# dmsuehir/unet_distributed

Hardware: AMD Instinct MI355X
Metric: images/sec (whole node) 2D UNet BraTS 128×128×4 at 1/2/4/8 MI355X; Dice parity (higher is better)
Workload: dtype bf16; 1 GPU; model=unet2d-transposed (base 32, depth 4, 7760385 params), global_batch=1024, per_gpu_batch=1024, img_size=128, in_channels=4, parallelism=dp1, backend=native

## Files before the change

unet_distributed_amd/csrc/kernels/conv_dw.hip:

```cpp
#include "common.h"
#include "conv_params.h"
#include "conv_epilogue.h"
#include "conv_win.h"
#include "head_grad.h"

namespace unet {
namespace {

constexpr int DW_NTHR = 256;
constexpr int DW_W = 128, DW_R = 2, DW_HR = DW_R + 2, DW_BM = DW_W * DW_R, DW_BN = 32;
constexpr int DW_HWP = (DW_W + 2 + 15) / 16 * 16;
constexpr int DW_PPR = DW_HWP / 16;
constexpr int DW_ROWB = DW_HWP * 64;
constexpr int DW_XI = DW_HR * DW_PPR;
constexpr int DW_WI = 9 * DW_BN / 16;
constexpr int DW_AI = DW_BM / 16;
constexpr int DW_WB = DW_WI * 1024, DW_XB = DW_XI * 1024, DW_AB = DW_AI * 1024;
constexpr int DW_KB = 6 * 32 * 4;
constexpr int DW_LDS = DW_WB + DW_XB + DW_AB + DW_KB;
static_assert(DW_BM * 64 + 4 * 2 * DW_BN * 4 <= 2 * DW_ROWB, "epilogue staging aliases two halo rows");
static_assert(4 * 64 * 16 * 4 <= DW_LDS, "slab reduction scratch");
constexpr int DW_HG = DW_HR * DW_HWP * 4;
constexpr int DW_HJ = DW_HG / DW_NTHR;
static_assert(DW_HG == DW_HJ * DW_NTHR, "whole granule passes");

template <int XF>
__device__ __forceinline__ void dw_dlogit(const ConvFwdParams& p, const float (&pr)[DW_HJ], const float (&tv)[DW_HJ],
                                          float (&dl)[DW_HJ]) {
  if constexpr (XF == 4) {
    const float I = p.hg.sums[0], St = p.hg.sums[1], Sp = p.hg.sums[2];
    const float a = -2.f / (2.f * I + 1.f), bb = 1.f / (St + Sp + 1.f);
    const float gs = p.hg.gscale ? *p.hg.gscale : 1.f;
#pragma unroll
    for (int j = 0; j < DW_HJ; ++j) dl[j] = head_dlogit(pr[j], tv[j], a, bb, p.hg.inv_total, p.hg.bce_w, gs);
  } else {
    const float gs = p.hg.gscale ? *p.hg.gscale : 1.f;
    const float al = -2.f * gs / (2.f * p.hg.sums[0] + 1.f);
    const float be = gs / (p.hg.sums[1] + p.hg.sums[2] + 1.f);
    const float ga = gs * p.hg.bce_w * p.hg.inv_total;
#pragma unroll
    for (int j = 0; j < DW_HJ; ++j) dl[j] = hn_dlogit(pr[j], tv[j], al, be, ga);
  }
}

template <int EPI, int XF, bool SEG = false>
__global__ void __launch_bounds__(DW_NTHR, 2) conv_dw_kernel(const ConvFwdParams p) {
  static_assert(XF == 0 || XF == 2 || XF == 3 || XF == 4,
                "plain dY, norm backward on load (of the normalised head), head gradient on load");
  constexpr int W = DW_W, R = DW_R, HR = DW_HR, ROWB = DW_ROWB, BN = DW_BN;
  constexpr int TM = 4, TN = 2, TC = 2, RW = 2, NCS = 4;
  __shared__ __attribute__((aligned(1024))) char smem[DW_LDS];
  char* Ws = smem;
  char* Xs = smem + DW_WB;
  char* As = Xs + DW_XB;

  const int tid = threadIdx.x, lane = tid & 63, wave = __builtin_amdgcn_readfirstlane(tid >> 6);
  const int H = p.OH;
  const int rows_total = p.N * H;
  const int Wf = SEG ? p.OW : W;
  const int M = rows_total * Wf;
  const int nrp = rows_total / R;
  const int nwin = nrp * (SEG ? Wf / W : 1);
  const int split = blockIdx.x;
  const int w_begin = (int)((long long)split * nwin / p.fw.nsplit);
  const int w_end = (int)((long long)(split + 1) * nwin / p.fw.nsplit);
  constexpr int OOB = 0x7fffffff;
  const int C = p.C1;
  const int Cx = p.fw.Cx;
  const int lslot = lane >> 2;
  const int lchunk = (lane & 3) ^ ((lslot >> 1) & 3);
  const int fsub = lane >> 4, fr = lane & 15;
  const int c0 = wave * 32;
  static_assert(DW_HR == 4 && DW_AI % 4 == 0, "one halo row per wave");
  const int dma_lane = ((lslot - 1) * 32 + lchunk * 8) * 2;
  const int xdma_lane = (lslot * 32 + lchunk * 8) * 2;

  {
    const __amdgpu_buffer_rsrc_t rsw = __builtin_amdgcn_make_buffer_rsrc((void*)p.wgt, (short)0, OOB, 0x00020000);
    const int wl = (lslot * p.Kpad + lchunk * 8) * 2;
#pragma unroll
    for (int q = 0; q < (DW_WI + 3) / 4; ++q) {
// ... 18 lines not shown
  const int G = lane >> 4, tq = (lane >> 2) & 3, pp = lane & 3;
  const int jw = wave & 1, sw0 = (wave >> 1) * 2;
  auto saddr = [](const int slot, const int col, const int ch) -> int {
    return slot * 64 + (((ch >> 3) ^ ((col >> 1) & 3)) << 4) + ((ch & 7) << 1);
  };
  const int kp0 = 16 * (G >> 1) + 4 * (G & 1) + tq;
  const int abase = saddr(kp0, kp0, 4 * pp);
  int dbase[3];
#pragma unroll
  for (int dw = 0; dw < 3; ++dw) {
    const int hc = kp0 + 2 - dw;
    dbase[dw] = saddr(hc, hc, 4 * pp) ^ (32 * jw);
  }
  auto tr8 = [&](const char* b0, const char* b1) -> h16x8 {
    const short4v lo = __builtin_amdgcn_ds_read_tr16_b64_v4i16(LDS_PTR(short4v, b0));
    const short4v hi = __builtin_amdgcn_ds_read_tr16_b64_v4i16(LDS_PTR(short4v, b1));
    const u32x2 l2 = __builtin_bit_cast(u32x2, lo), h2 = __builtin_bit_cast(u32x2, hi);
    const u32x4 v = {l2[0], l2[1], h2[0], h2[1]};
    return __builtin_bit_cast(h16x8, v);
  };

  f32x4 wacc[9][2];
#pragma unroll
  for (int t = 0; t < 9; ++t)
#pragma unroll
    for (int i = 0; i < 2; ++i) wacc[t][i] = (f32x4){0.f, 0.f, 0.f, 0.f};
  f32x4 bacc = (f32x4){0.f, 0.f, 0.f, 0.f};
  const u32x4 ones_u = {kOnes2, kOnes2, kOnes2, kOnes2};
  const h16x8 ones = __builtin_bit_cast(h16x8, ones_u);
  float* Ks = (float*)(As + DW_AB);
  const int kch = (tid & 3) * 8;
  int fl = 0;

  for (int win = w_begin; win < w_end; ++win) {
    const int seg = SEG ? win / nrp : 0;
    const int col0 = seg * W;
    const int g0 = (SEG ? win - seg * nrp : win) * R;
    const int grow0 = (g0 / H) * H;
    const bool top_in = (g0 % H) != 0, bot_in = ((g0 + R) % H) != 0;
    const bool carry = win > w_begin && top_in;
    if (carry) fl ^= 1;
    const int fo = fl * 2 * ROWB;
    const int k0 = carry ? 2 * DW_HWP * 4 : 0;
    const size_t img_px = (size_t)grow0 * Wf;
    const __amdgpu_buffer_rsrc_t rs1 = __builtin_amdgcn_make_buffer_rsrc(
        (void*)((const char*)p.src1 + img_px * C * 2), (short)0, OOB, 0x00020000);
    const __amdgpu_buffer_rsrc_t rsx = __builtin_amdgcn_make_buffer_rsrc(
        (void*)((const char*)p.fw.x + ((size_t)g0 * Wf + col0) * Cx * 2), (short)0, OOB, 0x00020000);
    u32x4 zv[XF == 2 ? DW_HJ : 1];
    float dl[XF >= 3 ? DW_HJ : 1];
    uint32_t hbits[XF == 4 ? DW_HJ : 1];
    float pr[XF >= 3 ? DW_HJ : 1], tv[XF >= 3 ? DW_HJ : 1];
    uint32_t okm = 0;
    if constexpr (XF >= 2) {
      float kv = 0.f;
      constexpr int NK = XF == 4 ? 32 : XF == 3 ? 192 : 96;
      if (tid < NK) {
        const int m = tid >> 5, c = tid & 31;
        if constexpr (XF == 4) {
          kv = p.hg.w[c];
        } else {
          const float* src = m == 0 ? p.xa : m == 1 ? p.xb : m == 2 ? p.xc : m == 3 ? p.hg.fa : m == 4 ? p.hg.fc : p.xa;
          const size_t ci = (size_t)(g0 / H) * p.xcs + c;
          kv = src[ci];
          if (XF == 3 && m == 5) kv *= p.hg.w[c];
        }
// ... 17 lines not shown
        if constexpr (XF == 2)
          zv[j] = __builtin_amdgcn_raw_buffer_load_b128(rsz, ok ? ((gr - grow0) * Wf + col) * C * 2 + kch * 2 : OOB,
                                                        0, 0);
      }
      if (tid < NK) Ks[tid] = kv;
    }
    __syncthreads();
    if constexpr (XF != 4) {
      const int hr = carry ? 2 + (wave >> 1) : wave;
      const int jlo = carry ? 5 * (wave & 1) : 0, jhi = carry && !(wave & 1) ? 5 : DW_PPR;
      const int gr = g0 - 1 + hr;
      const bool row_ok = (hr > 0 || top_in) && (hr < R + 1 || bot_in) && (unsigned)gr < (unsigned)rows_total;
      const int rowoff = ((gr - grow0) * Wf + col0) * C * 2;
      char* hdst = Xs + (hr ^ (2 * fl)) * ROWB;
#pragma unroll
      for (int j = 0; j < DW_PPR; ++j) {
        if (j < jlo || j >= jhi) continue;
        const bool ok = row_ok && (unsigned)(col0 + 16 * j + lslot - 1) < (unsigned)Wf && 16 * j + lslot <= W + 1;
        const int off = ok ? rowoff + dma_lane + j * 1024 : OOB;
        __builtin_amdgcn_raw_ptr_buffer_load_lds(rs1, (__attribute__((address_space(3))) void*)(hdst + j * 1024),
                                                 16, off, 0, 0, 0);
      }
    }
#pragma unroll
    for (int i = 0; i < DW_AI / 4; ++i) {
      const int k = 4 * wave + i;
      const int xo = SEG ? ((k >> 3) * Wf + 16 * (k & 7)) * Cx * 2 : k * 1024;
      __builtin_amdgcn_raw_ptr_buffer_load_lds(rsx, (__attribute__((address_space(3))) void*)(As + k * 1024), 16,
                                               xdma_lane + xo, 0, 0, 0);
    }
    __syncthreads();
    if constexpr (XF >= 3) dw_dlogit<XF>(p, pr, tv, dl);
    if constexpr (XF == 4) {
      float hw[8];
#pragma unroll
      for (int e = 0; e < 8; ++e) hw[e] = Ks[kch + e];
#pragma unroll
      for (int j = 0; j < DW_HJ; ++j) {
        const int k = k0 + tid + DW_NTHR * j;
        if (k >= DW_HG) continue;
        const int hr = k / (DW_HWP * 4), s = (k >> 2) - hr * DW_HWP;
        float o[8];
#pragma unroll
        for (int e = 0; e < 8; ++e) {
          const float v = dl[j] * hw[e];
          o[e] = ((hbits[j] >> e) & 1u) ? v : 0.f;
        }
        *(u32x4*)(Xs + ((hr ^ (2 * fl)) * DW_HWP + s) * 64 + 16 * ((tid & 3) ^ ((s >> 1) & 3))) = pack8(o);
      }
      __syncthreads();
    } else if constexpr (XF >= 2) {
      float ka[8], kb[8], kc[8], kf[8], kg[8];
#pragma unroll
      for (int e = 0; e < 8; ++e) {
        ka[e] = Ks[(XF == 3 ? 160 : 0) + kch + e];
        kb[e] = Ks[32 + kch + e];
        kc[e] = Ks[64 + kch + e];
        if constexpr (XF == 3) {
          kf[e] = Ks[96 + kch + e];
          kg[e] = Ks[128 + kch + e];
        }
      }
#pragma unroll
      for (int j = 0; j < DW_HJ; ++j) {
        const int k = k0 + tid + DW_NTHR * j;
        if (k >= DW_HG) continue;
        const int hr = k / (DW_HWP * 4), s = (k >> 2) - hr * DW_HWP;
        u32x4* slot = (u32x4*)(Xs + ((hr ^ (2 * fl)) * DW_HWP + s) * 64 + 16 * ((tid & 3) ^ ((s >> 1) & 3)));
        u32x4 v = {0u, 0u, 0u, 0u};
        if ((okm >> j) & 1u) {
          float gf[8], zf[8];
          if constexpr (XF == 3) {
            unpack8(*slot, zf);
#pragma unroll
            for (int e = 0; e < 8; ++e) {
              const float g = fmaf(kf[e], zf[e], kg[e]) > 0.f ? ka[e] * dl[j] : 0.f;
              gf[e] = g + fmaf(kb[e], zf[e], kc[e]);
            }
          } else {
            unpack8(zv[j], zf);
            unpack8(*slot, gf);
#pragma unroll
            for (int e = 0; e < 8; ++e) gf[e] = fmaf(ka[e], gf[e], fmaf(kb[e], zf[e], kc[e]));
          }
          v = pack8(gf);
        }
        *slot = v;
      }
      __syncthreads();
    }

#pragma unroll
    for (int st = 0; st < 2; ++st) {
      const int so = (sw0 + st) * 32 * 64;
      h16x8 xa[R][2];
#pragma unroll
      for (int y = 0; y < R; ++y)
#pragma unroll
        for (int i = 0; i < 2; ++i) {
          const int a = (abase ^ (32 * i)) + y * W * 64 + so;
          xa[y][i] = tr8(As + a, As + a + 512);
        }
#pragma unroll
      for (int hr = 0; hr < HR; ++hr) {
#pragma unroll
        for (int dw = 0; dw < 3; ++dw) {
          const int a = dbase[dw] + hr * ROWB + so + (hr < 2 ? fo : -fo);
          const h16x8 yb = tr8(Xs + a, Xs + a + 512);
          if (dw == 1 && hr >= 1 && hr <= R) bacc = mfma16(ones, yb, bacc);
#pragma unroll
          for (int dh = 0; dh < 3; ++dh) {
            const int y = hr - 2 + dh;
            if (y < 0 || y >= R) continue;
#pragma unroll
            for (int i = 0; i < 2; ++i) wacc[3 * dh + dw][i] = mfma16(xa[y][i], yb, wacc[3 * dh + dw][i]);
          }
        }
        __builtin_amdgcn_sched_barrier(0);
      }
    }

    f32x4 acc[TM][TN];
#pragma unroll
    for (int i = 0; i < TM; ++i)
#pragma unroll
      for (int j = 0; j < TN; ++j) acc[i][j] = (f32x4){0.f, 0.f, 0.f, 0.f};
#pragma unroll
    for (int dw = 0; dw < 3; ++dw) {
      h16x8 wf[3][TN];
#pragma unroll
      for (int dh = 0; dh < 3; ++dh)
#pragma unroll
        for (int j = 0; j < TN; ++j) wf[dh][j] = *(const h16x8*)(Ws + ((3 * dh + dw) * BN + 16 * j) * 64 + wbase);
#pragma unroll
      for (int hr = 0; hr < RW + 2; ++hr) {
#pragma unroll
        for (int ci = 0; ci < TC; ++ci) {
          const h16x8 xf = *(const h16x8*)(Xs + xbase[dw] + hr * ROWB + ci * 16 * 64 + (hr < 2 ? fo : -fo));
#pragma unroll
          for (int dh = 0; dh < 3; ++dh) {
            const int ri = hr - dh;
            if (ri < 0 || ri >= RW) continue;
#pragma unroll
            for (int j = 0; j < TN; ++j) acc[ri * TC + ci][j] = mfma16(wf[dh][j], xf, acc[ri * TC + ci][j]);
          }
        }
      }
    }
    __syncthreads();
    using Map = StripTiles<W, RW, TC, NCS>;
    if constexpr (SEG)
      conv_epilogue<DW_BM, BN, DW_BM / 4, BN, TM, TN, DW_NTHR, EPI, Map, W, W>(p, acc, Xs + fo, g0, 0, M, wave, 0,
                                                                              lane, tid, Wf, col0, win);
    else
      conv_epilogue<DW_BM, BN, DW_BM / 4, BN, TM, TN, DW_NTHR, EPI, Map, 0, W>(p, acc, Xs + fo, g0 * W, 0, M, wave, 0,
                                                                              lane, tid, 0, 0, win);
  }

  float* red = (float*)smem;
  const int row = p.fw.split_lo + split;
  const int n_base = lane & 15, m_base = 4 * (lane >> 4);
  auto reduce_store = [&](const f32x4 (&v4)[2], const int t) {
    __syncthreads();
    if (wave >= 2) {
#pragma unroll
      for (int i = 0; i < 2; ++i) *(f32x4*)(red + ((i * 2 + jw) * 64 + lane) * 4) = v4[i];
    }
    __syncthreads();
    if (wave < 2) {
#pragma unroll
      for (int i = 0; i < 2; ++i) {
        const f32x4 v = v4[i] + *(const f32x4*)(red + ((i * 2 + jw) * 64 + lane) * 4);
        if (t < 9) {
          float* dst = p.fw.slab + (((size_t)row * 9 + t) * Cx + m_base + 16 * i) * C + n_base + 16 * jw;
#pragma unroll
          for (int r = 0; r < 4; ++r) dst[(size_t)r * C] = v[r];
        } else if (i == 0 && lane < 16) {
          p.fw.bias_slab[(size_t)row * C + n_base + 16 * jw] = v[0];
        }
      }
    }
  };
#pragma unroll
  for (int t = 0; t < 9; ++t) reduce_store(wacc[t], t);
  const f32x4 bv[2] = {bacc, (f32x4){0.f, 0.f, 0.f, 0.f}};
  reduce_store(bv, 9);
}

}

const char* conv_dw_check(const ConvFwdParams& p) {
  if (!p.fw.x) return nullptr;
  const int ep = conv_epi_mode(p);
  const bool w_ok = p.OW == DW_W || (p.OW % DW_W == 0 && p.OW <= 8192);
  if (!w_ok || p.IW != p.OW || p.OH != p.IH || p.OH % DW_R || p.KD != 1 || p.OD != 1 || p.ID != 1 ||
      p.KH != 3 || p.KW != 3 || p.stride != 1 || p.pad != 1 || p.C1 != 32 || p.C2 || p.Cout != DW_BN ||
      p.D1 != p.Cout || p.fw.Cx != 32 || (ep != EPI_DGRAD && ep != EPI_DGRAD_NORM) || p.s2d ||
      p.ut.x || p.pool_dst || p.head_w || p.rev)
    return "conv_fwd: fused weight gradient needs a 2D 32 -> 32 channel data gradient on 128-wide rows";
  if (p.xform && (p.xform != 2 || !p.xa || !p.xb || !p.xc || !p.xz || (p.xcs != 0 && p.xcs != p.C1) || p.xout))
    return "conv_fwd: fused weight gradient: norm backward on load (xform 2) needs xa / xb / xc / xz, xcs 0 or C";
  if (p.hg.prob && p.xform && (p.xform != 2 || p.hg.bits || !p.hg.fa || !p.hg.fc || !p.hg.t || !p.hg.sums ||
                                !p.hg.w || p.route_gy))
    return "conv_fwd: fused weight gradient: the normalised head's gradient on load needs xform 2, "
           "fa / fc (no bits), t, sums, w";
  if (p.hg.prob && !p.xform && (!p.hg.bits || !p.hg.t || !p.hg.sums || !p.hg.w || p.route_gy || ep != EPI_DGRAD))
    return "conv_fwd: fused weight gradient: the head gradient on load needs bits, t, sums, w";
  if (!p.fw.slab || !p.fw.bias_slab || p.fw.nsplit < 1 || p.fw.split_lo < 0)
    return "conv_fwd: fused weight gradient needs slab / bias_slab and nsplit >= 1";
  if ((long long)p.OH * p.OW * 32 * 2 >= (1LL << 31) - 64) return "conv_fwd: one image exceeds 2 GiB";
  if (p.OW > DW_W && (p.xform || p.hg.prob || p.nz))
    return "conv_fwd: fused weight gradient on segmented rows: plain dY source, EPI_DGRAD only";
  return nullptr;
}

int conv_dw_grid(const ConvFwdParams& p) { return p.fw.nsplit; }

int conv_dw_stat_rows(const ConvFwdParams& p) { return p.N * p.OH / DW_R; }

hipError_t launch_conv_dw(const ConvFwdParams& p, hipStream_t s) {
  const int ep = conv_epi_mode(p);
  const dim3 grid(p.fw.nsplit), blk(DW_NTHR);
  if (p.OW > DW_W) {
    if (ep != EPI_DGRAD || p.xform || p.hg.prob) return hipErrorInvalidValue;
    UNET_LAUNCH((conv_dw_kernel<EPI_DGRAD, 0, true>), grid, blk, 0, s, p);
  } else if (ep == EPI_DGRAD && !p.xform && !p.hg.prob)
    UNET_LAUNCH((conv_dw_kernel<EPI_DGRAD, 0>), grid, blk, 0, s, p);
  else if (ep == EPI_DGRAD && !p.xform)
    UNET_LAUNCH((conv_dw_kernel<EPI_DGRAD, 4>), grid, blk, 0, s, p);
  else if (ep == EPI_DGRAD && p.xform == 2 && !p.hg.prob)
    UNET_LAUNCH((conv_dw_kernel<EPI_DGRAD, 2>), grid, blk, 0, s, p);
  else if (ep == EPI_DGRAD_NORM && !p.xform && !p.hg.prob)
    UNET_LAUNCH((conv_dw_kernel<EPI_DGRAD_NORM, 0>), grid, blk, 0, s, p);
  else if (ep == EPI_DGRAD_NORM && p.xform == 2 && !p.hg.prob)
    UNET_LAUNCH((conv_dw_kernel<EPI_DGRAD_NORM, 2>), grid, blk, 0, s, p);
  else if (ep == EPI_DGRAD_NORM && p.xform == 2)
    UNET_LAUNCH((conv_dw_kernel<EPI_DGRAD_NORM, 3>), grid, blk, 0, s, p);
  else
    return hipErrorInvalidValue;
  return launch_status();
}

}
```

unet_distributed_amd/csrc/kernels/conv_epilogue.h:

```cpp
#pragma once
#include "common.h"
#include "conv_params.h"

namespace unet {

struct PixCoord {
  int n, d, h, w;
};

__device__ __forceinline__ PixCoord decompose(int q, int OD, int OH, int OW) {
  PixCoord c;
  c.w = q % OW;
  int t = q / OW;
  c.h = t % OH;
  t /= OH;
  c.d = t % OD;
  c.n = t / OD;
  return c;
}

enum { EPI_GENERIC = 0, EPI_FWD = 1, EPI_DGRAD = 2, EPI_STATS = 3, EPI_DGRAD_NORM = 4 };

template <int BM, int BN, int NTHR = 256>
constexpr int epi_lds_bytes() {
// ... 16 lines not shown
}

__host__ __device__ inline const char* conv_norm_epi_check(const ConvFwdParams& p) {
  if (!p.stats && !p.nz) return nullptr;
  if (!p.stats) return "conv_fwd: nz (dgrad-norm epilogue) needs a stats buffer";
  if (p.relu || p.shuffle || p.drop_rate > 0.f || p.out_scale != 1.f || p.D1 != p.Cout || p.mask1 || p.mask2 ||
      p.head_w || p.relu_bits || p.mask_bits || (p.route_gy && !p.nz))
    return "conv_fwd: statistics epilogue takes no ReLU / dropout / shuffle / scale / split / mask / head";
  if (p.nz && (p.bias || !p.na || !p.nc || p.npix <= 0 || p.mask_scale1 != 1.f || (p.ncs != 0 && p.ncs != p.Cout)))
    return "conv_fwd: dgrad-norm epilogue needs na / nc / npix, no bias";
  return nullptr;
}

__host__ __device__ inline int conv_epi_mode(const ConvFwdParams& p) {
  if (p.nz) return EPI_DGRAD_NORM;
  if (p.stats) return EPI_STATS;
  if (p.shuffle || p.drop_rate > 0.f || p.out_scale != 1.f) return EPI_GENERIC;
  if (p.relu && p.D1 == p.Cout && !p.mask1 && !p.mask2 && p.mask_scale1 == 1.f) return EPI_FWD;
  if (!p.relu && !p.bias) return EPI_DGRAD;
  return EPI_GENERIC;
}

template <int WM>
struct LinearTiles {
  __device__ static int base(int wm, int i) { return wm * WM + i * 16; }
};
template <int W, int RW, int TC, int NCS>
struct StripTiles {
  __device__ static int base(int wave, int i) {
    return ((wave / NCS) * RW + i / TC) * W + (wave % NCS) * 16 * TC + (i % TC) * 16;
  }
};

template <int TN>
struct EpiConst {
  float bias[TN][4];
  float hw[8];
  float hb;
};

struct HeadWsum {
  float s[3][8];
  float u, v, w;
};
struct HeadT {
  float t[8];
  bool on;
};

template <int BM, int BN, int WM, int WN, int TM, int TN, int NTHR, int EPI = EPI_GENERIC,
          class MapM = LinearTiles<WM>, int SEGW = 0, int TROW = 0>
__device__ __forceinline__ HeadWsum conv_epilogue(const ConvFwdParams p, f32x4 (&acc)[TM][TN], char* smem,
                                                  const int m0, const int n0, const int M, const int wm,
                                                  const int wn, const int lane, const int tid,
                                                  const int pitch = 0, const int col0 = 0, const int stat_row = 0,
                                                  const EpiConst<TN>* ec = nullptr, const HeadT ht = HeadT{}) {
  HeadWsum hws;
#pragma unroll
  for (int k = 0; k < 3; ++k)
#pragma unroll
    for (int e = 0; e < 8; ++e) hws.s[k][e] = 0.f;
  hws.u = hws.v = hws.w = 0.f;
  auto qof = [&](int ml) -> int {
    if constexpr (SEGW > 0) return (m0 + ml / SEGW) * pitch + col0 + (ml % SEGW);
    else return m0 + ml;
  };
  constexpr bool ESWZ = BN == 32;
  constexpr int EPI_STRIDE = ESWZ ? 64 : (BN + 4) * 2;
  auto eoff = [](const int ml, const int chunk) -> int {
    return ESWZ ? ml * 64 + 16 * (chunk ^ ((ml >> 2) & 3)) : ml * EPI_STRIDE + 16 * chunk;
  };
  auto ehalf = [](const int ml, const int nl) -> int {
    return ESWZ ? ml * 64 + 16 * ((nl >> 3) ^ ((ml >> 2) & 3)) + ((2 * (nl & 7)) ^ (8 * ((ml >> 1) & 1)))
                : ml * EPI_STRIDE + 2 * nl;
  };
  auto eread = [&](const int ml, const int chunk) -> u32x4 {
    if constexpr (ESWZ) {
      const u32x4 v = *(const u32x4*)(smem + eoff(ml, chunk));
      return ((ml >> 1) & 1) ? (u32x4){v[2], v[3], v[0], v[1]} : v;
    } else {
      const u32x2 lo = *(const u32x2*)(smem + eoff(ml, chunk));
      const u32x2 hi = *(const u32x2*)(smem + eoff(ml, chunk) + 8);
      return (u32x4){lo[0], lo[1], hi[0], hi[1]};
    }
  };
  char* E = smem;
  float* SP = (float*)(smem + BM * EPI_STRIDE);
  constexpr bool G = EPI == EPI_GENERIC;
  constexpr bool kNormG = EPI == EPI_DGRAD_NORM;
// ... 23 lines not shown
      for (int i = 0; i < TM; ++i) {
        const int ml = MapM::base(wm, i) + (lane & 15);
        f32x2 a01 = (f32x2){acc[i][j][0], acc[i][j][1]} + b01;
        f32x2 a23 = (f32x2){acc[i][j][2], acc[i][j][3]} + b23;
        u32x2 pk;
        pk[0] = relu2h(pack2h(a01[0], a01[1]));
        pk[1] = relu2h(pack2h(a23[0], a23[1]));
        *(u32x2*)(E + ehalf(ml, nl)) = pk;
      }
      continue;
    }
#pragma unroll
    for (int i = 0; i < TM; ++i) {
      const int ml = MapM::base(wm, i) + (lane & 15);
      const int q = qof(ml);
      float v[4];
#pragma unroll
      for (int r = 0; r < 4; ++r) {
        float x = G ? acc[i][j][r] * p.out_scale + bsv[r] : acc[i][j][r] + bsv[r];
        if (kRelu) x = fmaxf(x, 0.f);
        if (kDrop) {
          const uint32_t h = drop_hash((uint64_t)q * p.Cout + n + r + p.drop_idx0, seed, p.salt);
          x = (h >= drop_thr) ? x * inv_keep : 0.f;
        }
        if (kMaskScale) x *= msc[r];
        v[r] = x;
      }
      u32x2 pk;
      pk[0] = pack2h(v[0], v[1]);
      pk[1] = pack2h(v[2], v[3]);
      *(u32x2*)(E + ehalf(ml, nl)) = pk;
    }
  }
  __syncthreads();

  constexpr int CPR = BN / 8;
  constexpr int NCHUNK = BM * CPR;
  auto stats_out = [&](float (&s1)[8], float (&s2)[8], int cb) {
#pragma unroll
    for (int o = CPR; o < 64; o <<= 1)
#pragma unroll
      for (int e = 0; e < 8; ++e) {
        s1[e] += __shfl_xor(s1[e], o, 64);
        s2[e] += __shfl_xor(s2[e], o, 64);
      }
    const int wv = tid >> 6;
    if ((tid & 63) < CPR) {
#pragma unroll
      for (int e = 0; e < 8; ++e) {
        SP[(wv * 2 + 0) * BN + cb * 8 + e] = s1[e];
        SP[(wv * 2 + 1) * BN + cb * 8 + e] = s2[e];
      }
    }
    __syncthreads();
    for (int t = tid; t < 2 * BN; t += NTHR) {
      const int mom = t / BN, c = t - mom * BN;
      float a = 0.f;
#pragma unroll
      for (int w = 0; w < NTHR / 64; ++w) a += SP[(w * 2 + mom) * BN + c];
      p.stats[((size_t)stat_row * 2 + mom) * p.Cout + n0 + c] = a;
    }
  };
  if constexpr (kStats) {
    static_assert(NCHUNK % NTHR == 0 && NTHR % CPR == 0 && CPR <= 64, "statistics tiling");
    constexpr int NIT = NCHUNK / NTHR, RPI = NTHR / CPR;
    const int cb = tid % CPR, ml0 = tid / CPR;
    const int n = n0 + cb * 8;
// ... 77 lines not shown
        for (int e = 0; e < 8; ++e)
          if (route_hit(cw, e, rk[it], d3)) g[e] += gg[e];
      }
#pragma unroll
      for (int e = 0; e < 8; ++e) {
        bool keep = fmaf(ca[e], z[e], cc[e]) > 0.f;
        if (drop) keep = keep && drop_hash((uint64_t)q * p.Cout + n + e, dseed, p.nd_salt) >= dthr;
        g[e] = keep ? g[e] * dscale : 0.f;
      }
      const u32x4 gv = pack8(g);
      *(u32x4*)(dst + (size_t)q * p.Cout + n) = gv;
      unpack8(gv, g);
#pragma unroll
      for (int e = 0; e < 8; ++e) {
        s1[e] += g[e];
        s2[e] = fmaf(g[e], z[e], s2[e]);
      }
    }
    stats_out(s1, s2, cb);
    return hws;
  }
  if constexpr (EPI == EPI_DGRAD && NCHUNK % NTHR == 0 && NTHR % CPR == 0) {
    constexpr int NIT = NCHUNK / NTHR, RPI = NTHR / CPR;
    const int cb = tid % CPR, ml0 = tid / CPR;
    const int n = n0 + cb * 8;
    const bool side1 = n < p.D1;
    const int rs = side1 ? p.D1 : p.Cout - p.D1;
    const int co = side1 ? n : n - p.D1;
    h16* dst = (h16*)(side1 ? p.dst1 : p.dst2);
    const h16* mk = (const h16*)(side1 ? p.mask1 : p.mask2);
    const bool mbit = (p.mask_bits >> (side1 ? 0 : 1)) & 1;
    u32x4 mv[NIT];
    uint32_t mb[NIT];
    if (mk) {
#pragma unroll
      for (int it = 0; it < NIT; ++it) {
        const int q = qof(ml0 + it * RPI);
        if (q < M) {
          if (mbit)
            mb[it] = ((const uint8_t*)mk)[((size_t)q * rs + co) >> 3];
          else
            mv[it] = *(const u32x4*)(mk + (size_t)q * rs + co);
        }
      }
    }
    const bool route = p.route_gy != nullptr, d3 = p.OD > 1;
    u32x4 rg[NIT];
    uint32_t rc[NIT], rk[NIT];
    if (route) {
      const int cpp = p.Cout >> 3;
#pragma unroll
      for (int it = 0; it < NIT; ++it) {
        const int q = qof(ml0 + it * RPI);
        if (q < M) {
          const size_t pq = route_pix(p, q, rk[it]);
          rc[it] = p.pool_code[pq * cpp + (n >> 3)];
          rg[it] = *(const u32x4*)((const h16*)p.route_gy + pq * p.Cout + n);
        }
      }
    }
#pragma unroll
    for (int it = 0; it < NIT; ++it) {
      const int ml = ml0 + it * RPI;
      const int q = qof(ml);
      if (q >= M) continue;
      u32x4 v = eread(ml, cb);
      if (mk) v = mbit ? keep_bits(v, mb[it]) : keep_pos(v, mv[it]);
      if (route) {
        float o[8], gg[8];
        unpack8(v, o);
        unpack8(rg[it], gg);
        const uint32_t cw = rc[it];
#pragma unroll
        for (int e = 0; e < 8; ++e)
          if (route_hit(cw, e, rk[it], d3)) o[e] += gg[e];
        v = pack8(o);
      }
      *(u32x4*)(dst + (size_t)q * rs + co) = v;
    }
    return hws;
  }
  const int Dt = kShuffle ? (p.Cout >> p.shuffle) : 0;
  constexpr bool kHeadable = EPI == EPI_FWD && BN == 32 && NTHR % CPR == 0;
  const bool kHead = kHeadable && p.head_w != nullptr;
  float hw[8], hb = 0.f;
  constexpr int HIT = kHeadable ? NCHUNK / NTHR : 1;
  static_assert(!kHeadable || (NCHUNK % NTHR == 0 && HIT % CPR == 0 && HIT <= 8), "fused head tiling");
  float hz[HIT];
  int hq[HIT];
#pragma unroll
  for (int k = 0; k < HIT; ++k) {
    hz[k] = 0.f;
    hq[k] = M;
  }
  if (kHeadable && kHead) {
#pragma unroll
    for (int e = 0; e < 8; ++e) hw[e] = ec ? ec->hw[e] : p.head_w[(tid % CPR) * 8 + e];
    hb = ec ? ec->hb : p.head_b[0];
  }
  constexpr int NITER = (NCHUNK + NTHR - 1) / NTHR;
// ... 145 lines not shown
```

unet_distributed_amd/csrc/kernels/conv_params.h:

```cpp
#pragma once
#include <stdint.h>

namespace unet_types {

bool dry_dispatch();

struct HeadGrad {
  const float* prob;
  const void* t;
  const float* sums;
  const float* w;
  const uint8_t* bits;
  const float* gscale;
  float inv_total, bce_w;
  const float* fa;
  const float* fc;
};

struct TconvSrc {
  const void* x;
  const void* w;
  const float* b;
  int C, kpad;
};

struct FusedWgrad {
  const void* x;
  float* slab;
  float* bias_slab;
  int Cx, nsplit, split_lo;
};

struct ConvFwdParams {
  int N, OD, OH, OW;
  int ID, IH, IW;
  int KD, KH, KW, stride, pad;
  int C1, C2;
  int up1;
  const void* src1;
  const void* src2;
  const void* wgt;
  const float* bias;
  int Cout;
  int relu;
  float out_scale;
  float drop_rate;
  uint32_t seed, salt;
  unsigned long long drop_idx0;
  const uint32_t* seed_ptr;
  void* dst1;
  void* dst2;
  int D1;
  const void* mask1;
  const void* mask2;
  float mask_scale1, mask_scale2;
  int shuffle;
  float* stats;
  const void* nz;
  const float* na;
  const float* nc;
  int ncs, npix;
  float nd_rate;
  uint32_t nd_salt;
// ... 128 lines not shown
```

unet_distributed_amd/csrc/runtime/bindings.cpp:

```cpp
#include <pybind11/pybind11.h>
#include <pybind11/stl.h>

#include <functional>
#include <stdexcept>
#include <string>
#include <tuple>
#include <vector>

#include "launch_api.h"

namespace py = pybind11;
using namespace unet;

namespace {

void check(hipError_t e, const char* what) {
  if (e != hipSuccess) throw std::runtime_error(std::string(what) + ": " + hipGetErrorString(e));
}

void check_msg(const char* msg) {
  if (msg) throw std::invalid_argument(msg);
}

template <typename T>
// ... 70 lines not shown
  p.mask_scale2 = get<float>(d, "mask_scale2", 1.f);
  p.shuffle = get<int>(d, "shuffle", 0);
  p.stats = (float*)getp(d, "stats");
  p.nz = getp(d, "nz");
  p.na = (const float*)getp(d, "na");
  p.nc = (const float*)getp(d, "nc");
  p.ncs = get<int>(d, "ncs", 0);
  p.npix = get<int>(d, "npix", 0);
  p.nd_rate = get<float>(d, "nd_rate", 0.f);
  p.nd_salt = get<uint32_t>(d, "nd_salt", 0u);
  p.pool_dst = const_cast<void*>(getp(d, "pool_dst"));
  p.pool_code = (uint32_t*)const_cast<void*>(getp(d, "pool_code"));
  p.relu_bits = (uint8_t*)const_cast<void*>(getp(d, "relu_bits"));
  p.mask_bits = get<int>(d, "mask_bits", 0);
  p.route_gy = getp(d, "route_gy");
  p.xform = get<int>(d, "xform", 0);
  p.xcs = get<int>(d, "xcs", 0);
  p.xa = (const float*)getp(d, "xa");
  p.xb = (const float*)getp(d, "xb");
  p.xc = (const float*)getp(d, "xc");
  p.xz = getp(d, "xz");
  p.s2d = get<int>(d, "s2d", 0);
  p.ut.x = getp(d, "ut_x");
  p.ut.w = getp(d, "ut_w");
  p.ut.b = (const float*)getp(d, "ut_b");
  p.ut.C = get<int>(d, "ut_C", 0);
  p.ut.kpad = get<int>(d, "ut_kpad", 0);
  p.fw.x = getp(d, "fw_x");
  p.fw.slab = (float*)const_cast<void*>(getp(d, "fw_slab"));
  p.fw.bias_slab = (float*)const_cast<void*>(getp(d, "fw_bias_slab"));
  p.fw.Cx = get<int>(d, "fw_Cx", 0);
  p.fw.nsplit = get<int>(d, "fw_nsplit", 0);
  p.fw.split_lo = get<int>(d, "fw_split_lo", 0);
  p.xout = const_cast<void*>(getp(d, "xout"));
  p.xd_rate = get<float>(d, "xd_rate", 0.f);
  p.xd_salt = get<uint32_t>(d, "xd_salt", 0u);
  p.xd_idx0 = get<unsigned long long>(d, "xd_idx0", 0ull);
  p.x2a = (const float*)getp(d, "x2a");
  p.x2b = (const float*)getp(d, "x2b");
  p.x2cs = get<int>(d, "x2cs", 0);
  p.tile = get<int>(d, "tile", 0);
  p.head_w = (const float*)getp(d, "head_w");
  p.head_b = (const float*)getp(d, "head_b");
  p.head_logit = (float*)const_cast<void*>(getp(d, "head_logit"));
  p.head_t = getp(d, "head_t");
  p.head_ws = (float*)const_cast<void*>(getp(d, "head_ws"));
  p.head_nostore = get<int>(d, "head_nostore", 0);
  p.hg = head_grad(d);
  if (!p.src1 || !p.wgt || (!p.dst1 && !(p.head_nostore && p.head_w)))
    throw std::invalid_argument("conv_fwd: src1/wgt/dst1 required");
  check_msg(conv_fwd_prepare(p));
  return p;
}

WgradParams wgrad_params(const py::dict& d) {
  WgradParams p{};
  p.N = get<int>(d, "N", 1);
  p.QD = get<int>(d, "QD", 1);
  p.QH = get<int>(d, "QH", 1);
  p.QW = get<int>(d, "QW", 1);
  p.AD = get<int>(d, "AD", 1);
  p.AH = get<int>(d, "AH", 1);
  p.AW = get<int>(d, "AW", 1);
  p.KD = get<int>(d, "KD", 1);
  p.KH = get<int>(d, "KH", 1);
  p.KW = get<int>(d, "KW", 1);
// ... 803 lines not shown
```

unet_distributed_amd/runtime/native_engine.py:

```python

import math
import os
from contextlib import nullcontext as _nullctx
from typing import Dict, List, Optional, Sequence, Tuple

import numpy as np
import torch

from .. import native
from ..models.spec import UNetSpec
from .params import FlatParams
from .plan_check import RecordingPlan



def _ptr(t: Optional[torch.Tensor]) -> Optional[int]:
    return None if t is None else int(t.data_ptr())


def _r64(k: int) -> int:
    return (k + 63) // 64 * 64


ENGINE_DEFAULTS = dict(dual_stream=1, fwd_streams=2, head_fuse=1, head_onload=1, tconv_fused=2, tconv_wa=1,
                       tconv_onload=1, fwd_offset=6, wg_target=512, dw_fuse=1, dw_wgs=512, win_pf=8, win_cp=1,
                       wg_pair=0, dz_split=0, head_wsum=1, xf_drop=0, wg_pf=1, win_cp3=2, skip_onload=1,
                       route3=1, tail3=0)


class Fusion:

    def __init__(self, doc, norm=None, dims=None, decoder=None, img=None, option=None, needs=(),
                 even_batch=False, cpad=None, when=None):
        self.doc, self.norm, self.dims, self.decoder, self.img = doc, norm, dims, decoder, img
        self.option, self.needs, self.even_batch, self.cpad, self.when = option, tuple(needs), even_batch, cpad, when

    def unmet(self, e) -> List[str]:
        out = []
        if self.norm is not None and e.spec.norm not in self.norm:
            out.append("norm=%s" % e.spec.norm)
        if self.dims is not None and e.dims not in self.dims:
            out.append("dims=%d" % e.dims)
        dec = "upsampling" if e.spec.use_upsampling else "transposed"
        if self.decoder is not None and dec not in self.decoder:
            out.append("decoder=%s" % dec)
        if self.img is not None and e.img not in self.img:
            out.append("img=%d" % e.img)
        if self.option is not None and not e.opts[self.option]:
            out.append("option %s=0" % self.option)
        if self.even_batch and e.B % 2:
            out.append("odd batch")
        if self.cpad is not None and e.cpad not in self.cpad:
            out.append("padded input channels %d" % e.cpad)
        if self.when is not None and not self.when(e):
            out.append("structure")
        return out


_ROW_IMGS = (16, 32, 64, 128)
FUSIONS: Dict[str, Fusion] = {
# ... 636 lines not shown
        b = self.bufs

        def half(t):
            return t.numel() * t.element_size() // 2

        mk = self.relu_bits.get(src1, b[src1]) if d.get("mask1") else None
        h1 = dict(d, N=self.B // 2)
        h2 = dict(h1, src1=d["src1"] + half(dy), dst1=d["dst1"] + half(b["d:" + src1]))
        if mk is not None:
            h2["mask1"] = d["mask1"] + half(mk)
        try:
            for h in (h1, h2):
                self.C.conv_fwd_grid(h)
        except ValueError:
            return None
        self._fusion_on("tail_halves", l.name)
        return h1, h2

    def _plan_dw_fuse(self, l, src1, skip, parts, wspec):
        if (not self._fusion_ok("dw_fused") or skip is not None or l.cin != 32 or l.cout != 32
                or wspec.get("kernel_out") or wspec["kd"].get("xform")
                or wspec["M1"] != 32 or wspec["M2"] or src1 not in self.bufs):
            return None
        nsplit = self.opts["dw_wgs"]
        b = self.bufs
        half = b[src1].numel() * b[src1].element_size() // len(parts)
        if len(parts) > 1 and parts[0].get("nz"):
            return None
        out = []
        for k, d in enumerate(parts):
            if d.get("route_gy") or (d.get("hg_prob") and len(parts) > 1):
                return None
            f = dict(d, rev=0, fw_x=_ptr(b[src1]) + k * half, fw_Cx=l.cin, fw_nsplit=nsplit, fw_split_lo=k * nsplit,
                     name=d["name"])
            if f.get("nz") and not self._restat_dgrad_norm(f, src1):
                return None
            try:
                if self.C.conv_fwd_grid(dict(f, fw_slab=1, fw_bias_slab=1)) != nsplit:
                    return None
            except ValueError:
                return None
            out.append(f)
        wspec["dw"] = dict(rows=nsplit * len(parts))
        self._fusion_on("dw_fused", l.name)
        if len(out) == 1 and l.name in self.norm_layers and self._fusion_ok("dz_onload", l.name):
            C = l.cout
            xf = dict(out[0], xform=2, src1=_ptr(b["d:" + l.name]), xz=_ptr(b["z:" + l.name]),
                      xa=_ptr(b["ca:" + l.name]), xb=_ptr(b["cb:" + l.name]), xc=_ptr(b["cc:" + l.name]),
                      xcs=0 if self.spec.norm == "batch" else C)
            if self._norm_head_loss and l.name == self.head_in:
                hg = self._head_grad_fields()
                hg.pop("hg_bits")
                xf.update(hg, src1=_ptr(b["z:" + l.name]), hg_fa=_ptr(b["fa:" + l.name]),
                          hg_fc=_ptr(b["fc:" + l.name]))
            try:
                ok = self.C.conv_fwd_grid(dict(xf, fw_slab=1, fw_bias_slab=1)) == nsplit
            except ValueError:
                ok = False
            if ok:
                out = [xf]
                self._dz_onload.add(l.name)
                self._fusion_on("dz_onload", l.name)
        return out

    def _dz_split_fields(self, l, src1, skip):
        if (not self._fusion_ok("dz_split") or skip is not None or l.name not in self.norm_layers
                or self.inputs.get(l.name, ("",))[1] != 1 or l.name in self._wa_chain_of
# ... 980 lines not shown
```

Before: 49450 images/sec.

## Software-pipeline fused conv dgrad/wgrad kernel with next-window prefetch

Adds a pipelined variant of the fused weight/data-gradient conv kernel for the plain and head-gradient paths. It issues the next window's input DMA and halo-row (or head probability/target/bit) loads into registers during the current window's MFMA work, replacing full syncthreads with LDS-only barriers. It also preloads mask bits before the compute so the epilogue does not fetch them late. The cost is higher register pressure at 2 waves per SIMD, plus a new code path gated on alignment and routing conditions.

```diff
diff --git a/unet_distributed_amd/csrc/kernels/conv_dw.hip b/unet_distributed_amd/csrc/kernels/conv_dw.hip
--- a/unet_distributed_amd/csrc/kernels/conv_dw.hip
+++ b/unet_distributed_amd/csrc/kernels/conv_dw.hip
@@ -43,10 +43,11 @@
   }
 }
 
-template <int EPI, int XF, bool SEG = false>
+template <int EPI, int XF, bool SEG = false, bool PIPE = false>
 __global__ void __launch_bounds__(DW_NTHR, 2) conv_dw_kernel(const ConvFwdParams p) {
   static_assert(XF == 0 || XF == 2 || XF == 3 || XF == 4,
                 "plain dY, norm backward on load (of the normalised head), head gradient on load");
+  static_assert(!PIPE || (EPI == EPI_DGRAD && (XF == 0 || XF == 4) && !SEG), "variants with a pipelined loop");
   constexpr int W = DW_W, R = DW_R, HR = DW_HR, ROWB = DW_ROWB, BN = DW_BN;
   constexpr int TM = 4, TN = 2, TC = 2, RW = 2, NCS = 4;
   __shared__ __attribute__((aligned(1024))) char smem[DW_LDS];
@@ -131,6 +132,87 @@
   const int kch = (tid & 3) * 8;
   int fl = 0;
 
+  auto wgrad_mfmas = [&](const int fo) {
+#pragma unroll
+    for (int st = 0; st < 2; ++st) {
+      const int so = (sw0 + st) * 32 * 64;
+      h16x8 xa[R][2];
+#pragma unroll
+      for (int y = 0; y < R; ++y)
+#pragma unroll
+        for (int i = 0; i < 2; ++i) {
+          const int a = (abase ^ (32 * i)) + y * W * 64 + so;
+          xa[y][i] = tr8(As + a, As + a + 512);
+        }
+#pragma unroll
+      for (int hr = 0; hr < HR; ++hr) {
+#pragma unroll
+        for (int dw = 0; dw < 3; ++dw) {
+          const int a = dbase[dw] + hr * ROWB + so + (hr < 2 ? fo : -fo);
+          const h16x8 yb = tr8(Xs + a, Xs + a + 512);
+          if (dw == 1 && hr >= 1 && hr <= R) bacc = mfma16(ones, yb, bacc);
+#pragma unroll
+          for (int dh = 0; dh < 3; ++dh) {
+            const int y = hr - 2 + dh;
+            if (y < 0 || y >= R) continue;
+#pragma unroll
+            for (int i = 0; i < 2; ++i) wacc[3 * dh + dw][i] = mfma16(xa[y][i], yb, wacc[3 * dh + dw][i]);
+          }
+        }
+        __builtin_amdgcn_sched_barrier(0);
+      }
+    }
+  };
+  auto dgrad_mfmas = [&](f32x4 (&acc)[TM][TN], const int fo) {
+#pragma unroll
+    for (int i = 0; i < TM; ++i)
+#pragma unroll
+      for (int j = 0; j < TN; ++j) acc[i][j] = (f32x4){0.f, 0.f, 0.f, 0.f};
+#pragma unroll
+    for (int dw = 0; dw < 3; ++dw) {
+      h16x8 wf[3][TN];
+#pragma unroll
+      for (int dh = 0; dh < 3; ++dh)
+#pragma unroll
+        for (int j = 0; j < TN; ++j) wf[dh][j] = *(const h16x8*)(Ws + ((3 * dh + dw) * BN + 16 * j) * 64 + wbase);
+#pragma unroll
+      for (int hr = 0; hr < RW + 2; ++hr) {
+#pragma unroll
+        for (int ci = 0; ci < TC; ++ci) {
+          const h16x8 xf = *(const h16x8*)(Xs + xbase[dw] + hr * ROWB + ci * 16 * 64 + (hr < 2 ? fo : -fo));
+#pragma unroll
+          for (int dh = 0; dh < 3; ++dh) {
+            const int ri = hr - dh;
+            if (ri < 0 || ri >= RW) continue;
+#pragma unroll
+            for (int j = 0; j < TN; ++j) acc[ri * TC + ci][j] = mfma16(wf[dh][j], xf, acc[ri * TC + ci][j]);
+          }
+        }
+      }
+    }
+  };
+  auto form_head_dy = [&](const int k0, const int fl, const auto& dl, const auto& hbits) {
+    if constexpr (XF == 4) {
+      float hw[8];
+#pragma unroll
+      for (int e = 0; e < 8; ++e) hw[e] = Ks[kch + e];
+#pragma unroll
+      for (int j = 0; j < DW_HJ; ++j) {
+        const int k = k0 + tid + DW_NTHR * j;
+        if (k >= DW_HG) continue;
+        const int hr = k / (DW_HWP * 4), s = (k >> 2) - hr * DW_HWP;
+        float o[8];
+#pragma unroll
+        for (int e = 0; e < 8; ++e) {
+          const float v = dl[j] * hw[e];
+          o[e] = ((hbits[j] >> e) & 1u) ? v : 0.f;
+        }
+        *(u32x4*)(Xs + ((hr ^ (2 * fl)) * DW_HWP + s) * 64 + 16 * ((tid & 3) ^ ((s >> 1) & 3))) = pack8(o);
+      }
+    }
+  };
+
+  if constexpr (!PIPE)
   for (int win = w_begin; win < w_end; ++win) {
     const int seg = SEG ? win / nrp : 0;
     const int col0 = seg * W;
@@ -214,22 +296,7 @@
     __syncthreads();
     if constexpr (XF >= 3) dw_dlogit<XF>(p, pr, tv, dl);
     if constexpr (XF == 4) {
-      float hw[8];
-#pragma unroll
-      for (int e = 0; e < 8; ++e) hw[e] = Ks[kch + e];
-#pragma unroll
-      for (int j = 0; j < DW_HJ; ++j) {
-        const int k = k0 + tid + DW_NTHR * j;
-        if (k >= DW_HG) continue;
-        const int hr = k / (DW_HWP * 4), s = (k >> 2) - hr * DW_HWP;
-        float o[8];
-#pragma unroll
-        for (int e = 0; e < 8; ++e) {
-          const float v = dl[j] * hw[e];
-          o[e] = ((hbits[j] >> e) & 1u) ? v : 0.f;
-        }
-        *(u32x4*)(Xs + ((hr ^ (2 * fl)) * DW_HWP + s) * 64 + 16 * ((tid & 3) ^ ((s >> 1) & 3))) = pack8(o);
-      }
+      form_head_dy(k0, fl, dl, hbits);
       __syncthreads();
     } else if constexpr (XF >= 2) {
       float ka[8], kb[8], kc[8], kf[8], kg[8];
@@ -272,63 +339,9 @@
       __syncthreads();
     }
 
-#pragma unroll
-    for (int st = 0; st < 2; ++st) {
-      const int so = (sw0 + st) * 32 * 64;
-      h16x8 xa[R][2];
-#pragma unroll
-      for (int y = 0; y < R; ++y)
-#pragma unroll
-        for (int i = 0; i < 2; ++i) {
-          const int a = (abase ^ (32 * i)) + y * W * 64 + so;
-          xa[y][i] = tr8(As + a, As + a + 512);
-        }
-#pragma unroll
-      for (int hr = 0; hr < HR; ++hr) {
-#pragma unroll
-        for (int dw = 0; dw < 3; ++dw) {
-          const int a = dbase[dw] + hr * ROWB + so + (hr < 2 ? fo : -fo);
-          const h16x8 yb = tr8(Xs + a, Xs + a + 512);
-          if (dw == 1 && hr >= 1 && hr <= R) bacc = mfma16(ones, yb, bacc);
-#pragma unroll
-          for (int dh = 0; dh < 3; ++dh) {
-            const int y = hr - 2 + dh;
-            if (y < 0 || y >= R) continue;
-#pragma unroll
-            for (int i = 0; i < 2; ++i) wacc[3 * dh + dw][i] = mfma16(xa[y][i], yb, wacc[3 * dh + dw][i]);
-          }
-        }
-        __builtin_amdgcn_sched_barrier(0);
-      }
-    }
-
+    wgrad_mfmas(fo);
     f32x4 acc[TM][TN];
-#pragma unroll
-    for (int i = 0; i < TM; ++i)
-#pragma unroll
-      for (int j = 0; j < TN; ++j) acc[i][j] = (f32x4){0.f, 0.f, 0.f, 0.f};
-#pragma unroll
-    for (int dw = 0; dw < 3; ++dw) {
-      h16x8 wf[3][TN];
-#pragma unroll
-      for (int dh = 0; dh < 3; ++dh)
-#pragma unroll
-        for (int j = 0; j < TN; ++j) wf[dh][j] = *(const h16x8*)(Ws + ((3 * dh + dw) * BN + 16 * j) * 64 + wbase);
-#pragma unroll
-      for (int hr = 0; hr < RW + 2; ++hr) {
-#pragma unroll
-        for (int ci = 0; ci < TC; ++ci) {
-          const h16x8 xf = *(const h16x8*)(Xs + xbase[dw] + hr * ROWB + ci * 16 * 64 + (hr < 2 ? fo : -fo));
-#pragma unroll
-          for (int dh = 0; dh < 3; ++dh) {
-            const int ri = hr - dh;
-            if (ri < 0 || ri >= RW) continue;
-#pragma unroll
-            for (int j = 0; j < TN; ++j) acc[ri * TC + ci][j] = mfma16(wf[dh][j], xf, acc[ri * TC + ci][j]);
-          }
-        }
-      }
-    }
+    dgrad_mfmas(acc, fo);
     __syncthreads();
     using Map = StripTiles<W, RW, TC, NCS>;
     if constexpr (SEG)
@@ -337,6 +350,156 @@
     else
       conv_epilogue<DW_BM, BN, DW_BM / 4, BN, TM, TN, DW_NTHR, EPI, Map, 0, W>(p, acc, Xs + fo, g0 * W, 0, M, wave, 0,
                                                                               lane, tid, 0, 0, win);
+  }
+
+  if constexpr (PIPE) {
+    constexpr int NPF = 5;
+    static_assert(2 * NPF >= DW_PPR && NPF * DW_NTHR >= DW_HG / 2, "two halo rows in NPF passes");
+    auto x_dma = [&](const int w) {
+      const __amdgpu_buffer_rsrc_t rsx = __builtin_amdgcn_make_buffer_rsrc(
+          (void*)((const char*)p.fw.x + (size_t)w * R * W * Cx * 2), (short)0, OOB, 0x00020000);
+#pragma unroll
+      for (int i = 0; i < DW_AI / 4; ++i) {
+        const int k = 4 * wave + i;
+        __builtin_amdgcn_raw_ptr_buffer_load_lds(rsx, (__attribute__((address_space(3))) void*)(As + k * 1024), 16,
+                                                 xdma_lane + k * 1024, 0, 0, 0);
+      }
+    };
+    auto head_loads = [&](const int g0, const bool top_in, const bool bot_in, const int k0, auto& pr, auto& tv,
+                          auto& hb, uint32_t& okm) {
+      constexpr int NJ = sizeof(pr) / sizeof(pr[0]);
+      okm = 0;
+#pragma unroll
+      for (int j = 0; j < NJ; ++j) {
+        const int k = k0 + tid + DW_NTHR * j;
+        const int hr = k / (DW_HWP * 4), s = (k >> 2) - hr * DW_HWP;
+        const int gr = g0 - 1 + hr, col = s - 1;
+        const bool ok = k < DW_HG && (hr > 0 || top_in) && (hr < R + 1 || bot_in) &&
+                        (unsigned)gr < (unsigned)rows_total && (unsigned)col < (unsigned)W && s <= W + 1;
+        okm |= (ok ? 1u : 0u) << j;
+        const int pix = ok ? gr * W + col : 0;
+        pr[j] = p.hg.prob[pix];
+        tv[j] = ((const uint32_t*)p.hg.t)[pix >> 1];
+        hb[j] = ((const uint32_t*)p.hg.bits)[pix];
+      }
+    };
+    u32x4 nhv[XF == 0 ? NPF : 1];
+    float npr[XF == 4 ? NPF : 1];
+    uint32_t ntv[XF == 4 ? NPF : 1], nhb[XF == 4 ? NPF : 1], nokm = 0;
+#pragma unroll
+    for (int i = 0; i < (XF == 0 ? NPF : 1); ++i) nhv[i] = (u32x4){0u, 0u, 0u, 0u};
+#pragma unroll
+    for (int i = 0; i < (XF == 4 ? NPF : 1); ++i) {
+      npr[i] = 0.f;
+      ntv[i] = nhb[i] = 0u;
+    }
+    float hd_a = 0.f, hd_b = 0.f, hd_gs = 1.f;
+    if constexpr (XF == 4) {
+      const float I = p.hg.sums[0], St = p.hg.sums[1], Sp = p.hg.sums[2];
+      hd_a = -2.f / (2.f * I + 1.f);
+      hd_b = 1.f / (St + Sp + 1.f);
+      hd_gs = p.hg.gscale ? *p.hg.gscale : 1.f;
+    }
+    if constexpr (XF == 4) {
+      if (tid < 32) Ks[tid] = p.hg.w[tid];
+    }
+    if (w_begin < w_end) x_dma(w_begin);
+    const int pj0 = NPF * (wave & 1);
+
+    for (int win = w_begin; win < w_end; ++win) {
+      const int g0 = win * R;
+      const int grow0 = (g0 / H) * H;
+      const bool top_in = (g0 % H) != 0, bot_in = ((g0 + R) % H) != 0;
+      const bool carry = win > w_begin && top_in;
+      if (carry) fl ^= 1;
+      const int fo = fl * 2 * ROWB;
+      const int k0 = carry ? 2 * DW_HWP * 4 : 0;
+      const __amdgpu_buffer_rsrc_t rs1 = __builtin_amdgcn_make_buffer_rsrc(
+          (void*)((const char*)p.src1 + (size_t)grow0 * W * C * 2), (short)0, OOB, 0x00020000);
+      lds_barrier();
+      __builtin_amdgcn_s_waitcnt(kWaitVm0);
+      float pr[XF == 4 ? DW_HJ : 1];
+      uint32_t tv[XF == 4 ? DW_HJ : 1], hb[XF == 4 ? DW_HJ : 1], okm = nokm;
+      if constexpr (XF == 0) {
+        if (!carry) {
+          const int gr = g0 - 1 + wave;
+          const bool row_ok = (wave > 0 || top_in) && (wave < R + 1 || bot_in) && (unsigned)gr < (unsigned)rows_total;
+          const int rowoff = (gr - grow0) * W * C * 2;
+          char* hdst = Xs + (wave ^ (2 * fl)) * ROWB;
+#pragma unroll
+          for (int j = 0; j < DW_PPR; ++j) {
+            const bool ok = row_ok && (unsigned)(16 * j + lslot - 1) < (unsigned)W;
+            __builtin_amdgcn_raw_ptr_buffer_load_lds(rs1, (__attribute__((address_space(3))) void*)(hdst + j * 1024),
+                                                     16, ok ? rowoff + dma_lane + j * 1024 : OOB, 0, 0, 0);
+          }
+          __builtin_amdgcn_s_waitcnt(kWaitVm0);
+        } else {
+          char* hdst = Xs + ((2 + (wave >> 1)) ^ (2 * fl)) * ROWB;
+#pragma unroll
+          for (int i = 0; i < NPF; ++i)
+            if (pj0 + i < DW_PPR) *(u32x4*)(hdst + (pj0 + i) * 1024 + lane * 16) = nhv[i];
+        }
+      } else {
+        if (!carry) {
+          head_loads(g0, top_in, bot_in, 0, pr, tv, hb, okm);
+        } else {
+#pragma unroll
+          for (int j = 0; j < DW_HJ; ++j) {
+            pr[j] = j < NPF ? npr[j < NPF ? j : 0] : 0.f;
+            tv[j] = j < NPF ? ntv[j < NPF ? j : 0] : 0u;
+            hb[j] = j < NPF ? nhb[j < NPF ? j : 0] : 0u;
+          }
+        }
+        float dl[DW_HJ];
+        uint32_t hbits[DW_HJ];
+#pragma unroll
+        for (int j = 0; j < DW_HJ; ++j) {
+          const int par = (((k0 + tid + DW_NTHR * j) >> 2) - 1) & 1;
+          hbits[j] = ((okm >> j) & 1u) ? (hb[j] >> (8 * (tid & 3))) & 0xffu : 0u;
+          dl[j] = head_dlogit(pr[j], bits2f((uint16_t)(tv[j] >> (16 * par))), hd_a, hd_b, p.hg.inv_total,
+                              p.hg.bce_w, hd_gs);
+        }
+        form_head_dy(k0, fl, dl, hbits);
+      }
+      uint32_t mb[DW_BM * (BN / 8) / DW_NTHR];
+#pragma unroll
+      for (int it = 0; it < DW_BM * (BN / 8) / DW_NTHR; ++it) mb[it] = 0u;
+      if (p.mask1) epi_mask_bits_load<DW_BM, BN, DW_NTHR>(p, g0 * W, 0, tid, mb);
+      lds_barrier();
+
+      wgrad_mfmas(fo);
+
+#pragma unroll
+      for (int it = 0; it < DW_BM * (BN / 8) / DW_NTHR; ++it) asm volatile("" : "+v"(mb[it]));
+      lds_barrier();
+      if (win + 1 < w_end) {
+        x_dma(win + 1);
+        const int g0n = g0 + R;
+        if ((g0n % H) != 0) {
+          const bool bot_n = ((g0n + R) % H) != 0;
+          if constexpr (XF == 0) {
+            const int hr = 2 + (wave >> 1), gr = g0n - 1 + hr;
+            const bool row_ok = (hr < R + 1 || bot_n) && (unsigned)gr < (unsigned)rows_total;
+            const int rowoff = (gr - grow0) * W * C * 2;
+#pragma unroll
+            for (int i = 0; i < NPF; ++i) {
+              const int j = pj0 + i;
+              const bool ok = row_ok && j < DW_PPR && (unsigned)(16 * j + lslot - 1) < (unsigned)W;
+              nhv[i] = __builtin_amdgcn_raw_buffer_load_b128(rs1, ok ? rowoff + dma_lane + j * 1024 : OOB, 0, 0);
+            }
+          } else {
+            head_loads(g0n, true, bot_n, 2 * DW_HWP * 4, npr, ntv, nhb, nokm);
+          }
+        }
+      }
+
+      f32x4 acc[TM][TN];
+      dgrad_mfmas(acc, fo);
+      lds_barrier();
+      conv_epilogue<DW_BM, BN, DW_BM / 4, BN, TM, TN, DW_NTHR, EPI, StripTiles<W, RW, TC, NCS>, 0, W>(
+          p, acc, Xs + fo, g0 * W, 0, M, wave, 0, lane, tid, 0, 0, win, nullptr, HeadT{}, mb);
+    }
+    __builtin_amdgcn_s_waitcnt(kWaitVm0);
   }
 
   float* red = (float*)smem;
@@ -403,14 +566,22 @@
 hipError_t launch_conv_dw(const ConvFwdParams& p, hipStream_t s) {
   const int ep = conv_epi_mode(p);
   const dim3 grid(p.fw.nsplit), blk(DW_NTHR);
+  const bool pipe = p.fw.pipe && (!p.mask1 || (p.mask_bits & 1)) && !p.route_gy &&
+                    (((uintptr_t)p.hg.t | (uintptr_t)p.hg.bits) & 3) == 0;
   if (p.OW > DW_W) {
     if (ep != EPI_DGRAD || p.xform || p.hg.prob) return hipErrorInvalidValue;
     UNET_LAUNCH((conv_dw_kernel<EPI_DGRAD, 0, true>), grid, blk, 0, s, p);
-  } else if (ep == EPI_DGRAD && !p.xform && !p.hg.prob)
-    UNET_LAUNCH((conv_dw_kernel<EPI_DGRAD, 0>), grid, blk, 0, s, p);
-  else if (ep == EPI_DGRAD && !p.xform)
-    UNET_LAUNCH((conv_dw_kernel<EPI_DGRAD, 4>), grid, blk, 0, s, p);
-  else if (ep == EPI_DGRAD && p.xform == 2 && !p.hg.prob)
+  } else if (ep == EPI_DGRAD && !p.xform && !p.hg.prob) {
+    if (pipe)
+      UNET_LAUNCH((conv_dw_kernel<EPI_DGRAD, 0, false, true>), grid, blk, 0, s, p);
+    else
+      UNET_LAUNCH((conv_dw_kernel<EPI_DGRAD, 0>), grid, blk, 0, s, p);
+  } else if (ep == EPI_DGRAD && !p.xform) {
+    if (pipe)
+      UNET_LAUNCH((conv_dw_kernel<EPI_DGRAD, 4, false, true>), grid, blk, 0, s, p);
+    else
+      UNET_LAUNCH((conv_dw_kernel<EPI_DGRAD, 4>), grid, blk, 0, s, p);
+  } else if (ep == EPI_DGRAD && p.xform == 2 && !p.hg.prob)
     UNET_LAUNCH((conv_dw_kernel<EPI_DGRAD, 2>), grid, blk, 0, s, p);
   else if (ep == EPI_DGRAD_NORM && !p.xform && !p.hg.prob)
     UNET_LAUNCH((conv_dw_kernel<EPI_DGRAD_NORM, 0>), grid, blk, 0, s, p);
diff --git a/unet_distributed_amd/csrc/kernels/conv_epilogue.h b/unet_distributed_amd/csrc/kernels/conv_epilogue.h
--- a/unet_distributed_amd/csrc/kernels/conv_epilogue.h
+++ b/unet_distributed_amd/csrc/kernels/conv_epilogue.h
@@ -72,6 +72,14 @@
   }
 };
 
+constexpr int kWaitVm0 = 0x0f70, kWaitLgkm0 = 0xc07f;
+__device__ __forceinline__ void lds_barrier() {
+  asm volatile("" ::: "memory");
+  __builtin_amdgcn_s_waitcnt(kWaitLgkm0);
+  __builtin_amdgcn_s_barrier();
+  asm volatile("" ::: "memory");
+}
+
 template <int TN>
 struct EpiConst {
   float bias[TN][4];
@@ -88,13 +96,25 @@
   bool on;
 };
 
+template <int BM, int BN, int NTHR>
+__device__ __forceinline__ void epi_mask_bits_load(const ConvFwdParams& p, const int m0, const int n0, const int tid,
+                                                   uint32_t (&mb)[BM * (BN / 8) / NTHR]) {
+  constexpr int CPR = BN / 8, NIT = BM * CPR / NTHR, RPI = NTHR / CPR;
+  static_assert(BM * CPR % NTHR == 0 && NTHR % CPR == 0, "whole chunk passes");
+  const int co = n0 + (tid % CPR) * 8, ml0 = tid / CPR;
+#pragma unroll
+  for (int it = 0; it < NIT; ++it)
+    mb[it] = ((const uint8_t*)p.mask1)[((size_t)(m0 + ml0 + it * RPI) * p.D1 + co) >> 3];
+}
+
 template <int BM, int BN, int WM, int WN, int TM, int TN, int NTHR, int EPI = EPI_GENERIC,
           class MapM = LinearTiles<WM>, int SEGW = 0, int TROW = 0>
 __device__ __forceinline__ HeadWsum conv_epilogue(const ConvFwdParams p, f32x4 (&acc)[TM][TN], char* smem,
                                                   const int m0, const int n0, const int M, const int wm,
                                                   const int wn, const int lane, const int tid,
                                                   const int pitch = 0, const int col0 = 0, const int stat_row = 0,
-                                                  const EpiConst<TN>* ec = nullptr, const HeadT ht = HeadT{}) {
+                                                  const EpiConst<TN>* ec = nullptr, const HeadT ht = HeadT{},
+                                                  const uint32_t* pmb = nullptr) {
   HeadWsum hws;
 #pragma unroll
   for (int k = 0; k < 3; ++k)
@@ -184,7 +204,10 @@
       *(u32x2*)(E + ehalf(ml, nl)) = pk;
     }
   }
-  __syncthreads();
+  if (pmb)
+    lds_barrier();
+  else
+    __syncthreads();
 
   constexpr int CPR = BN / 8;
   constexpr int NCHUNK = BM * CPR;
@@ -328,7 +351,10 @@
     const bool mbit = (p.mask_bits >> (side1 ? 0 : 1)) & 1;
     u32x4 mv[NIT];
     uint32_t mb[NIT];
-    if (mk) {
+    if (mk && pmb) {
+#pragma unroll
+      for (int it = 0; it < NIT; ++it) mb[it] = pmb[it];
+    } else if (mk) {
 #pragma unroll
       for (int it = 0; it < NIT; ++it) {
         const int q = qof(ml0 + it * RPI);
@@ -340,7 +366,7 @@
         }
       }
     }
-    const bool route = p.route_gy != nullptr, d3 = p.OD > 1;
+    const bool route = !pmb && p.route_gy != nullptr, d3 = p.OD > 1;
     u32x4 rg[NIT];
     uint32_t rc[NIT], rk[NIT];
     if (route) {
@@ -361,7 +387,7 @@
       const int q = qof(ml);
       if (q >= M) continue;
       u32x4 v = eread(ml, cb);
-      if (mk) v = mbit ? keep_bits(v, mb[it]) : keep_pos(v, mv[it]);
+      if (mk) v = (mbit || pmb) ? keep_bits(v, mb[it]) : keep_pos(v, mv[it]);
       if (route) {
         float o[8], gg[8];
         unpack8(v, o);
diff --git a/unet_distributed_amd/csrc/kernels/conv_params.h b/unet_distributed_amd/csrc/kernels/conv_params.h
--- a/unet_distributed_amd/csrc/kernels/conv_params.h
+++ b/unet_distributed_amd/csrc/kernels/conv_params.h
@@ -29,6 +29,7 @@
   float* slab;
   float* bias_slab;
   int Cx, nsplit, split_lo;
+  int pipe;
 };
 
 struct ConvFwdParams {
diff --git a/unet_distributed_amd/csrc/runtime/bindings.cpp b/unet_distributed_amd/csrc/runtime/bindings.cpp
--- a/unet_distributed_amd/csrc/runtime/bindings.cpp
+++ b/unet_distributed_amd/csrc/runtime/bindings.cpp
@@ -126,6 +126,7 @@
   p.fw.Cx = get<int>(d, "fw_Cx", 0);
   p.fw.nsplit = get<int>(d, "fw_nsplit", 0);
   p.fw.split_lo = get<int>(d, "fw_split_lo", 0);
+  p.fw.pipe = get<int>(d, "fw_pipe", 1);
   p.xout = const_cast<void*>(getp(d, "xout"));
   p.xd_rate = get<float>(d, "xd_rate", 0.f);
   p.xd_salt = get<uint32_t>(d, "xd_salt", 0u);
diff --git a/unet_distributed_amd/runtime/native_engine.py b/unet_distributed_amd/runtime/native_engine.py
--- a/unet_distributed_amd/runtime/native_engine.py
+++ b/unet_distributed_amd/runtime/native_engine.py
@@ -25,7 +25,7 @@
 ENGINE_DEFAULTS = dict(dual_stream=1, fwd_streams=2, head_fuse=1, head_onload=1, tconv_fused=2, tconv_wa=1,
                        tconv_onload=1, fwd_offset=6, wg_target=512, dw_fuse=1, dw_wgs=512, win_pf=8, win_cp=1,
                        wg_pair=0, dz_split=0, head_wsum=1, xf_drop=0, wg_pf=1, win_cp3=2, skip_onload=1,
-                       route3=1, tail3=0)
+                       route3=1, tail3=0, dw_pipe=1)
 
 
 class Fusion:
@@ -728,7 +728,7 @@
             if d.get("route_gy") or (d.get("hg_prob") and len(parts) > 1):
                 return None
             f = dict(d, rev=0, fw_x=_ptr(b[src1]) + k * half, fw_Cx=l.cin, fw_nsplit=nsplit, fw_split_lo=k * nsplit,
-                     name=d["name"])
+                     fw_pipe=self.opts["dw_pipe"], name=d["name"])
             if f.get("nz") and not self._restat_dgrad_norm(f, src1):
                 return None
             try:
```

Result: faster. 50360 images/sec, median of 6 (+1.8%).
